# MIT-REALM/gcbfplus

Hardware: NVIDIA H100
Metric: env-steps/sec (agents x envs x steps/s) DoubleIntegrator n=512 (higher is better)
Workload: dtype f32

## Files before the change

gcbfplus_b200/csrc/gemm_tc_prod.cuh:

```cuda
#pragma once
#include "gemm_tc.cuh"
#include "gnn.cuh"

namespace gcbf {
namespace tc {

struct ProdArgs {
    gcbf_env_desc d;
    const float *W1, *b1, *agent, *goal, *hits;
    const int32_t *edge_recv, *edge_src;
    int clip_all;
};

struct ChainArgs {
    const float* bias_g;
    const float* avec;
    const float* cst;
    float* logits;
};

constexpr int L1_FLOATS = 9 * 256;

template <int ED>
__device__ __forceinline__ void load_l1_table(float* sW, const float* W1, const float* b1, int tid, int nthreads) {
    for (int i = tid; i < ED * 256; i += nthreads) sW[i] = W1[i];
    for (int i = tid; i < 3 * 256; i += nthreads) {
        const int t = i / 256, c = i % 256;
        sW[(ED + t) * 256 + c] = W1[(ED + t) * 256 + c] + W1[(ED + 3 + 2) * 256 + c] + b1[c];
    }
}

template <int ED>
__device__ __forceinline__ void produce_l1_kblock(uint8_t* st, int r, int half, int kb, bool row_ok, const float* sW,
                                                  const float (&f)[ED], int stype) {
#pragma unroll
    for (int cc = 0; cc < 4; ++cc) {
        const int c = half * 4 + cc;
        float v[4] = {0.f, 0.f, 0.f, 0.f};
        if (row_ok) {
            const int n = kb * BK + c * 4;
#pragma unroll
            for (int j = 0; j < 4; ++j) {
                float y = sW[(ED + stype) * 256 + n + j];
#pragma unroll
                for (int q = 0; q < ED; ++q) y = fmaf(f[q], sW[q * 256 + n + j], y);
                v[j] = fmaxf(y, 0.f);
            }
        }
        float4 h, l;
        split_tf32(make_float4(v[0], v[1], v[2], v[3]), h, l);
        const int off = swz(r, c);
        *reinterpret_cast<float4*>(st + off) = h;
        *reinterpret_cast<float4*>(st + PLANE + off) = l;
    }
}

__device__ __forceinline__ void drain_msg(const float (&d)[64], uint8_t* smem, int g, int wt, const float* bias,
                                          float* msg, int n_valid) {
    const int r0 = 64 * g + frag_row0(wt);
#pragma unroll
    for (int i = 0; i < 64; i += 2) {
        const int r = r0 + 8 * ((i >> 1) & 1);
        const int c = frag_col(wt, i);
        const float2 o = make_float2(d[i] + bias[c], d[i + 1] + bias[c + 1]);
        if (r < n_valid) *reinterpret_cast<float2*>(msg + (size_t)r * 128 + c) = o;
        const float2 h = make_float2(rn_tf32(o.x), rn_tf32(o.y));
        const float2 l = make_float2(rn_tf32(o.x - h.x), rn_tf32(o.y - h.y));
        const int off = (c >> 5) * 32768 + swz(r, (c & 31) >> 2) + (c & 3) * 4;
        *reinterpret_cast<float2*>(smem + off) = h;
        *reinterpret_cast<float2*>(smem + off + 16384) = l;
    }
}

__device__ __forceinline__ void chain_kblock(float (&d)[64], uint8_t* smem, int g, int kb2, int slot) {
    const uint32_t a_hi = smem_u32(smem + kb2 * 32768) + g * WG_ROWS_BYTES;
    const uint32_t b_hi = smem_u32(smem + 2 * STG + slot * 32768);
    mma_kblock(d, a_hi, a_hi + 16384, b_hi, b_hi + 16384, kb2 == 0);
}

template <int KIND>
__device__ __forceinline__ void edge_row_setup(const ProdArgs& pa, int m, bool row_ok, float (&f)[EnvTraits<KIND>::ED],
                                               int& stype) {
    using T = EnvTraits<KIND>;
    constexpr int ED = T::ED, SD = T::SD;
    const int A_tot = pa.d.n_graphs * pa.d.n_agents;
#pragma unroll
    for (int c = 0; c < ED; ++c) f[c] = 0.f;
    stype = 0;
    if (row_ok) {
        const int a = min(max(pa.edge_recv[m], 0), A_tot - 1);
        const int code = min(pa.edge_src[m], A_tot - 1);
        float er[ED], es[ED], coef, nrm;
        edge_state_dev<KIND>(pa.agent + (size_t)a * SD, er);
        sender_state_dev<KIND>(code, a, pa.d.n_hits, pa.agent, pa.goal, pa.hits, es);
        edge_feat_dev<KIND>(er, es, pa.clip_all || code == -1, pa.d.comm_radius, f, &coef, &nrm);
        stype = (code >= 0) ? 2 : ((code == -1) ? 1 : 0);
    }
}

template <int ED>
__device__ __forceinline__ void edge_tile_mainloop(float (&d)[64], uint8_t* smem, uint64_t* full, uint64_t* empty,
                                                   uint32_t& it, int g, int r, int half, bool row_ok, const float* sW,
                                                   const float (&f)[ED], int stype) {
#pragma unroll
    for (int i = 0; i < 64; ++i) d[i] = 0.f;
    for (int kb = 0; kb < 8; ++kb, ++it) {
        const int s = it % STAGES;
        uint8_t* st = smem + s * STG;
        produce_l1_kblock<ED>(st, r, half, kb, row_ok, sW, f, stype);
        fence_async_smem();
        bar_wg(g);
        mbar_wait(&full[s], (it / STAGES) & 1);
        wg_fence();
        const uint32_t a_hi = smem_u32(st) + g * WG_ROWS_BYTES;
        mma_kblock(d, a_hi, a_hi + PLANE, smem_u32(st) + 2 * PLANE, smem_u32(st) + 3 * PLANE, kb == 0);
        wg_commit();
        wg_wait<1>();
        if (kb > 0) mbar_arrive(&empty[(it - 1) % STAGES]);
    }
    wg_wait<0>();
    mbar_arrive(&empty[(it - 1) % STAGES]);
}

template <int KIND>
__global__ void __launch_bounds__(THREADS_NN, 1)
edge_chain_kernel(const __grid_constant__ CUtensorMap tmBh, const __grid_constant__ CUtensorMap tmBl,
                  const __grid_constant__ CUtensorMap tmB2h, const __grid_constant__ CUtensorMap tmB2l,
                  const __grid_constant__ ProdArgs pa, const float* __restrict__ bias, float* __restrict__ C,
                  const int32_t* __restrict__ m_ptr, const int m_cap, const ChainArgs ch) {
    constexpr int ED = EnvTraits<KIND>::ED;
    extern __shared__ uint8_t smem_raw[];
    uint8_t* smem = smem_align1024(smem_raw);
    uint64_t* bars = reinterpret_cast<uint64_t*>(smem + STAGES * STG);
    uint64_t* full = bars;
    uint64_t* empty = bars + 3;
    uint64_t* b2_full = bars + 6;
    uint64_t* b2_empty = bars + 8;
    uint64_t* main_done = bars + 10;
    uint64_t* t2f = bars + 11;
    float* sW = reinterpret_cast<float*>(smem + STAGES * STG + 256);

    const int warp = threadIdx.x >> 5, lane = threadIdx.x & 31;
    if (threadIdx.x == 0) {
        for (int s = 0; s < 3; ++s) {
            mbar_init(&full[s], 1);
            mbar_init(&empty[s], CONSUMERS);
        }
        for (int i = 0; i < 2; ++i) {
            mbar_init(&b2_full[i], 1);
            mbar_init(&b2_empty[i], CONSUMERS);
        }
        mbar_init(main_done, CONSUMERS);
        mbar_init(t2f, CONSUMERS);
        asm volatile("fence.mbarrier_init.release.cluster;" ::: "memory");
    }
    load_l1_table<ED>(sW, pa.W1, pa.b1, threadIdx.x, blockDim.x);
    __syncthreads();
    const int M = min(*m_ptr, m_cap);
    const int n_tiles = (M + BM - 1) / BM;

    if (warp == 8) {
        if (lane == 0) {
            uint32_t it = 0, tc_ = 0;
            for (int tile = blockIdx.x; tile < n_tiles; tile += gridDim.x, ++tc_) {
                if (tc_ > 0) mbar_wait(t2f, (tc_ - 1) & 1);
                for (int kb = 0; kb < 8; ++kb, ++it) {
                    const int s = it % STAGES;
                    mbar_wait(&empty[s], ((it / STAGES) & 1) ^ 1);
                    uint8_t* st = smem + s * STG;
                    mbar_expect_tx(&full[s], 2 * PLANE);
                    tma_load_2d(st + 2 * PLANE, &tmBh, &full[s], kb * BK, 0);
                    tma_load_2d(st + 3 * PLANE, &tmBl, &full[s], kb * BK, 0);
                }
                mbar_wait(main_done, tc_ & 1);
                for (int kb2 = 0; kb2 < 4; ++kb2) {
                    const uint32_t j2 = tc_ * 4 + kb2, slot = j2 & 1, use = j2 >> 1;
                    mbar_wait(&b2_empty[slot], (use & 1) ^ 1);
                    uint8_t* sl = smem + 2 * STG + slot * 32768;
                    mbar_expect_tx(&b2_full[slot], 32768);
                    tma_load_2d(sl, &tmB2h, &b2_full[slot], kb2 * BK, 0);
                    tma_load_2d(sl + 16384, &tmB2l, &b2_full[slot], kb2 * BK, 0);
                }
            }
        }
        return;
    }
    const int g = warp >> 2, wt = threadIdx.x & 127;
    const int r = 64 * g + (wt & 63), half = wt >> 6;
    uint32_t it = 0, tc_ = 0;
    for (int tile = blockIdx.x; tile < n_tiles; tile += gridDim.x, ++tc_) {
        const int m0 = tile * BM;
        float f[ED];
        int stype;
        edge_row_setup<KIND>(pa, m0 + r, m0 + r < M, f, stype);
        float d[64];
        edge_tile_mainloop<ED>(d, smem, full, empty, it, g, r, half, m0 + r < M, sW, f, stype);
        mbar_arrive(main_done);
        bar_consumers();
        drain_msg(d, smem, g, wt, bias, C + (size_t)m0 * 128, M - m0);
        fence_async_smem();
        bar_wg(g);
        float d2[64];
#pragma unroll
        for (int i = 0; i < 64; ++i) d2[i] = 0.f;
        for (int kb2 = 0; kb2 < 4; ++kb2) {
            const uint32_t j2 = tc_ * 4 + kb2, slot = j2 & 1, use = j2 >> 1;
            mbar_wait(&b2_full[slot], use & 1);
            wg_fence();
            chain_kblock(d2, smem, g, kb2, slot);
            wg_commit();
            wg_wait<0>();
            mbar_arrive(&b2_empty[slot]);
        }
        float q[2][1];
        frag_relu_dot<1>(d2, ch.bias_g, ch.avec, 1, 1, wt, q);
        if ((lane & 3) == 0) {
            const int rr = m0 + 64 * g + frag_row0(wt);
            if (rr < M) ch.logits[rr] = q[0][0] + ch.cst[0];
            if (rr + 8 < M) ch.logits[rr + 8] = q[1][0] + ch.cst[0];
        }
        mbar_arrive(t2f);
        bar_consumers();
    }
}

constexpr int PROD_SMEM = STAGES * STG + 256 + L1_FLOATS * 4 + 1024;

inline int32_t launch_edge_msg(const gcbf_env_desc* d, const float* W1, const float* b1, const float* agent,
                               const float* goal, const float* hits, const int32_t* edge_recv,
                               const int32_t* edge_src, const int32_t* counters, int clip_all, const float* Bt_hi,
                               const float* Bt_lo, const float* bias, float* msg, cudaStream_t st,
                               const float* gate_Bt_hi, const float* gate_Bt_lo, const ChainArgs& chain) {
    if (!counters) {
        set_error("launch_edge_msg: the chained gate GEMM needs the device edge counter");
        return -1;
    }
    ProdArgs pa;
    memset(&pa, 0, sizeof(pa));
    pa.d = *d;
    pa.W1 = W1; pa.b1 = b1; pa.agent = agent; pa.goal = goal; pa.hits = hits;
    pa.edge_recv = edge_recv; pa.edge_src = edge_src; pa.clip_all = clip_all;
    const int K = 256, N = 128;
    CUtensorMap tmB, tmBl, tmG, tmGl;
    if (int32_t r = make_map(&tmB, Bt_hi, N, K, N)) return r;
    if (int32_t r = make_map(&tmBl, Bt_lo, N, K, N)) return r;
    if (int32_t r = make_map(&tmG, gate_Bt_hi, 128, 128, 128)) return r;
    if (int32_t r = make_map(&tmGl, gate_Bt_lo, 128, 128, 128)) return r;
    const int grid = min((d->edge_cap + BM - 1) / BM, sm_count());
    GCBF_DISPATCH_ENV(d->env_kind, {
        auto kern = edge_chain_kernel<KIND>;
        static bool attr_done = false;
        if (!attr_done) {
            cudaFuncSetAttribute(kern, cudaFuncAttributeMaxDynamicSharedMemorySize, PROD_SMEM);
            attr_done = true;
        }
        kern<<<grid, THREADS_NN, PROD_SMEM, st>>>(tmB, tmBl, tmG, tmGl, pa, bias, msg, counters, d->edge_cap, chain);
        count_launch();
        return check_launch("edge_chain_kernel");
// ... 7 lines not shown
```

gcbfplus_b200/csrc/rollout_persist.cu:

```cuda
#include <stdlib.h>

#include "gemm_tc_prod.cuh"
#include "geometry_dev.cuh"
#include "gnn.cuh"

namespace gcbf {
namespace rp {
using namespace tc;

constexpr int PT = 512;
constexpr int PW = PT / 32;
constexpr int STG = 65536;
constexpr int MAX_N = 512;
constexpr int MAX_OBS = 32;

enum { B_FULL = 0, B_EMPTY = 3, B_B2F = 6, B_B2E = 8, B_MAIN = 10, B_T2F = 11, B_COUNT = 12 };

constexpr int PNU = 2;
enum {
    K_B23 = 0,
    K_BIAS_G = 128,
    K_AVEC = 256,
    K_BU1 = 384,
    K_BU1ROW = 640,
// ... 5 lines not shown
};

struct PArgs {
    gcbf_env_desc d;
    int T, cap_env, C;
    const float *W1, *b1, *b23, *bias_g, *avec, *cst, *b_u1, *b_u1row, *buh, *ho, *bho;
    const float *goal, *obstacles, *ray_table;
    float *agent, *hits, *actions, *rewards, *costs;
    int32_t* counters;
    int32_t *row_start, *row_deg, *edge_recv, *edge_src;
    float *msg, *logit, *ag, *v1, *z;
    unsigned long long* prof;
    int soft;
    unsigned* gbar;
};

__device__ __forceinline__ unsigned long long gtime() {
    unsigned long long t;
    asm volatile("mov.u64 %0, %%globaltimer;" : "=l"(t));
    return t;
}
__device__ __forceinline__ void cluster_sync_all() {
    __syncwarp();
    asm volatile("barrier.cluster.arrive.release.aligned;\n\tbarrier.cluster.wait.acquire.aligned;" ::: "memory");
}
__device__ __forceinline__ void soft_group_sync(unsigned* ctr, unsigned target) {
    __syncthreads();
    if (threadIdx.x == 0) {
        __threadfence();
        atomicAdd(ctr, 1u);
        unsigned v;
        const unsigned long long t0 = global_ns();
        do {
            asm volatile("ld.acquire.gpu.global.u32 %0, [%1];" : "=r"(v) : "l"(ctr) : "memory");
            if (v < target && global_ns() - t0 > MBAR_TIMEOUT_NS) __trap();
        } while (v < target);
        __threadfence();
    }
    __syncthreads();
}
__device__ __forceinline__ void fence_async_global() { asm volatile("fence.proxy.async.global;" ::: "memory"); }
template <int KIND>
__global__ void __launch_bounds__(PT, 1)
rollout_persist_kernel(const __grid_constant__ PArgs P, const __grid_constant__ CUtensorMap tmW23h,
                       const __grid_constant__ CUtensorMap tmW23l, const __grid_constant__ CUtensorMap tmA1h,
                       const __grid_constant__ CUtensorMap tmA1l, const __grid_constant__ CUtensorMap tmU1h,
                       const __grid_constant__ CUtensorMap tmU1l, const __grid_constant__ CUtensorMap tmUHh,
                       const __grid_constant__ CUtensorMap tmUHl, const __grid_constant__ CUtensorMap tmAG,
                       const __grid_constant__ CUtensorMap tmV1) {
    using TR = EnvTraits<KIND>;
    constexpr int SD = TR::SD, ED = TR::ED, NU = TR::NU, PD = TR::PD;
    static_assert(PD == 2 && NU == PNU, "persistent rollout kernel: 2-D environments");
    constexpr int OBW = 16, OBS2 = OBS2D;
    constexpr int A_BYTES = 16384, B_BYTES = 16384;
    extern __shared__ uint8_t smem_raw[];
    uint8_t* smem = smem_align1024(smem_raw);
    uint64_t* bars = reinterpret_cast<uint64_t*>(smem + 3 * STG);
    int* s_tot = reinterpret_cast<int*>(smem + 3 * STG + 256 + 16);
    float* sW = reinterpret_cast<float*>(smem + 3 * STG + 512);
    float* sst = sW + 7 * 256;
    float* sobs = sst + MAX_N * 4;
    float* stab = sobs + MAX_OBS * OBS2;
    unsigned* sbits = reinterpret_cast<unsigned*>(stab + 64);
    int* s_off = reinterpret_cast<int*>(sbits + 64 * 16);
    unsigned* s_hb = reinterpret_cast<unsigned*>(s_off + 72);
    float* s_red = reinterpret_cast<float*>(s_hb + 64);
    float* sk = s_red + 3 * PW;

    const gcbf_env_desc& d = P.d;
    const int tid = threadIdx.x, warp = tid >> 5, lane = tid & 31;
    const int C = P.C;
    const bool soft = P.soft != 0;
    const int rank = (int)(blockIdx.x % C);
    const int env = blockIdx.x / C;
    const int L = soft ? 2 : C;
    const int lrank = rank % L, grp = rank / L;
    unsigned n_sync = 0;
#define SYNC_LOCAL() cluster_sync_all()
#define SYNC_ENV()                                                     \
    do {                                                               \
        if (soft) {                                                    \
            ++n_sync;                                                  \
            soft_group_sync(P.gbar + env, n_sync * (unsigned)C);       \
        } else {                                                       \
            cluster_sync_all();                                        \
        }                                                              \
    } while (0)
    const int N = d.n_agents, E = d.n_graphs, O = d.n_obs, R = d.n_hits, cap = P.cap_env;
    const int A_tot = E * N;
    const int APC = (N + C - 1) / C;
    const int a_lo = min(rank * APC, N), a_hi = min(a_lo + APC, N);
    const int n_words = (N + 31) / 32;
    const size_t env_e0 = (size_t)env * cap;
    const int env_a0 = env * N;
    const int seg_cap = cap / (C / L);
    const int seg_off = grp * seg_cap;
    const int ga_lo = min(grp * L * APC, N), ga_hi = min(ga_lo + L * APC, N);

    if (tid == 0) {
        for (int s = 0; s < 3; ++s) {
            mbar_init(&bars[B_FULL + s], 1);
            mbar_init(&bars[B_EMPTY + s], CONSUMERS);
        }
        for (int i = 0; i < 2; ++i) {
            mbar_init(&bars[B_B2F + i], 1);
            mbar_init(&bars[B_B2E + i], CONSUMERS);
        }
        mbar_init(&bars[B_MAIN], CONSUMERS);
        mbar_init(&bars[B_T2F], CONSUMERS);
        asm volatile("fence.mbarrier_init.release.cluster;" ::: "memory");
    }
    for (int i = tid; i < ED * 256; i += PT) sW[i] = P.W1[i];
    for (int i = tid; i < 3 * 256; i += PT) {
        const int t = i / 256, c = i % 256;
        sW[(ED + t) * 256 + c] = P.W1[(ED + t) * 256 + c] + P.W1[(ED + 3 + 2) * 256 + c] + P.b1[c];
    }
    auto stage = [&](int off, const float* src, int n) {
        for (int i = tid; i < n; i += PT) sk[off + i] = src[i];
    };
    stage(K_B23, P.b23, 128);
    stage(K_BIAS_G, P.bias_g, 128);
    stage(K_AVEC, P.avec, 128);
    stage(K_BU1, P.b_u1, 256);
    stage(K_BU1ROW, P.b_u1row, 256);
    stage(K_BUH, P.buh, 256);
    stage(K_HO, P.ho, 256 * NU);
    stage(K_BHO, P.bho, NU);
    stage(K_CST, P.cst, 1);
    if (O > 0) {
        const float* ob = P.obstacles + (d.obs_per_graph ? (size_t)env * O * OBW : 0);
        for (int i = tid; i < O * OBW; i += PT) sobs[(i / OBW) * OBS2 + (i % OBW)] = ob[i];
    }
    for (int i = tid; i < d.n_rays * PD; i += PT) stab[i] = P.ray_table[i];
    __syncthreads();
    derive_far_fields(sobs, O, d.comm_radius, tid, PT);
    uint32_t it = 0;
    uint32_t ne = 0;
    int M_cur = 0;
    SYNC_LOCAL();
    if (P.prof != nullptr && rank == 0 && tid == 0) P.prof[(size_t)(P.T + 1) * 8 + 2 * env] = gtime();

    for (int t = -1; t < P.T; ++t) {
        const int b = t & 1;
        const float* agent_t = P.agent + (size_t)max(t, 0) * A_tot * SD;
        const float* hits_t = P.hits + (size_t)max(t, 0) * A_tot * R * PD;
        const int32_t* rs_t = P.row_start + (size_t)b * A_tot;
        const int32_t* rd_t = P.row_deg + (size_t)b * A_tot;
        const int32_t* er_t = P.edge_recv + (size_t)b * E * cap;
        const int32_t* es_t = P.edge_src + (size_t)b * E * cap;
        const bool stamp = P.prof != nullptr && blockIdx.x == 0 && tid == 0;
        unsigned long long* pr = P.prof + (size_t)(t + 1) * 8;
        if (stamp) pr[0] = gtime();
        if (t >= 0) {
            const int n_tiles = (M_cur + BM - 1) / BM;
            const int my_tiles = (n_tiles > lrank) ? (n_tiles - lrank + L - 1) / L : 0;
            const size_t seg_e0 = env_e0 + seg_off;
            if (warp == 0) {
                if (lane == 0) {
                    uint32_t it_l = it, ne_l = ne;
                    for (int tile = lrank; tile < n_tiles; tile += L, ++ne_l) {
                        if (ne_l > 0) mbar_wait(&bars[B_T2F], (ne_l - 1) & 1);
                        for (int kb = 0; kb < 8; ++kb, ++it_l) {
                            const int s = it_l % 3;
                            mbar_wait(&bars[B_EMPTY + s], ((it_l / 3) & 1) ^ 1);
                            uint8_t* st = smem + s * STG;
                            mbar_expect_tx(&bars[B_FULL + s], 2 * B_BYTES);
                            tma_load_2d(st + 2 * A_BYTES, &tmW23h, &bars[B_FULL + s], kb * BK, 0);
                            tma_load_2d(st + 2 * A_BYTES + B_BYTES, &tmW23l, &bars[B_FULL + s], kb * BK, 0);
                        }
                        mbar_wait(&bars[B_MAIN], ne_l & 1);
                        for (int kb2 = 0; kb2 < 4; ++kb2) {
                            const uint32_t j2 = ne_l * 4 + kb2, slot = j2 & 1, use = j2 >> 1;
                            mbar_wait(&bars[B_B2E + slot], (use & 1) ^ 1);
                            uint8_t* sl = smem + 2 * STG + slot * 32768;
                            mbar_expect_tx(&bars[B_B2F + slot], 32768);
                            tma_load_2d(sl, &tmA1h, &bars[B_B2F + slot], kb2 * BK, 0);
                            tma_load_2d(sl + 16384, &tmA1l, &bars[B_B2F + slot], kb2 * BK, 0);
                        }
                    }
                }
            } else if (warp >= 8) {
                const int g = (warp - 8) >> 2, wt = tid & 127;
                const int r = 64 * g + (wt & 63), half = wt >> 6;
                uint32_t it_l = it, ne_l = ne;
                for (int tile = lrank; tile < n_tiles; tile += L, ++ne_l) {
                    const int ml = tile * BM + r;
                    const bool row_ok = ml < M_cur;
                    float f[ED];
                    int stype = 0;
#pragma unroll
                    for (int c = 0; c < ED; ++c) f[c] = 0.f;
                    if (row_ok) {
                        const int a = min(max(er_t[seg_e0 + ml], env_a0), env_a0 + N - 1);
                        const int code = min(es_t[seg_e0 + ml], env_a0 + N - 1);
                        float er[ED], es[ED], coef, nrm;
                        edge_state_dev<KIND>(sst + (size_t)(a - env_a0) * SD, er);
                        if (code >= 0) edge_state_dev<KIND>(sst + (size_t)(max(code, env_a0) - env_a0) * SD, es);
                        else sender_state_dev<KIND>(code, a, R, agent_t, P.goal, hits_t, es);
                        edge_feat_dev<KIND>(er, es, code == -1, d.comm_radius, f, &coef, &nrm);
                        stype = (code >= 0) ? 2 : ((code == -1) ? 1 : 0);
                    }
                    float dacc[64];
                    edge_tile_mainloop<ED>(dacc, smem, &bars[B_FULL], &bars[B_EMPTY], it_l, g, r, half, row_ok, sW, f, stype);
                    mbar_arrive(&bars[B_MAIN]);
                    bar_consumers();
                    drain_msg(dacc, smem, g, wt, sk + K_B23, P.msg + (seg_e0 + (size_t)tile * BM) * 128, M_cur - tile * BM);
                    fence_async_smem();
                    bar_wg(g);
                    float d2[64];
#pragma unroll
                    for (int i = 0; i < 64; ++i) d2[i] = 0.f;
                    for (int kb2 = 0; kb2 < 4; ++kb2) {
                        const uint32_t j2 = ne_l * 4 + kb2, slot = j2 & 1, use = j2 >> 1;
                        mbar_wait(&bars[B_B2F + slot], use & 1);
                        wg_fence();
                        chain_kblock(d2, smem, g, kb2, slot);
                        wg_commit();
                        wg_wait<0>();
                        mbar_arrive(&bars[B_B2E + slot]);
                    }
                    float q[2][1];
                    frag_relu_dot<1>(d2, sk + K_BIAS_G, sk + K_AVEC, 1, 1, wt, q);
                    if ((lane & 3) == 0) {
                        const int rr = tile * BM + 64 * g + frag_row0(wt);
                        if (rr < M_cur) P.logit[seg_e0 + rr] = q[0][0] + sk[K_CST];
                        if (rr + 8 < M_cur) P.logit[seg_e0 + rr + 8] = q[1][0] + sk[K_CST];
                    }
                    mbar_arrive(&bars[B_T2F]);
                    bar_consumers();
                }
            }
            it += 8u * my_tiles;
            ne += my_tiles;
            SYNC_LOCAL();
            if (stamp) pr[1] = gtime();

            for (int il = a_lo + warp; il < a_hi; il += PW) {
                const int a = env_a0 + il;
                const int rs = rs_t[a];
                int rd = rd_t[a];
                if (rs < 0 || rs + rd > cap) rd = 0;
                *reinterpret_cast<float4*>(P.ag + (size_t)a * 128 + lane * 4) =
                    aggregate_logits(rs, rd, P.logit + env_e0, P.msg + env_e0 * 128, lane);
            }
            fence_async_global();
            SYNC_LOCAL();
            if (stamp) pr[2] = gtime();

            const int n_items = ((ga_hi - ga_lo + BM - 1) / BM) * 2;
            const int my_items = (n_items > lrank) ? (n_items - lrank + L - 1) / L : 0;
            float* z_t = P.z + (size_t)(t & 1) * 2 * A_tot * 4;
#pragma unroll 1
            for (int ph2 = 0; ph2 < 2; ++ph2) {
                const int nkb = ph2 == 0 ? 4 : 8;
                const CUtensorMap* tmA = ph2 == 0 ? &tmAG : &tmV1;
                const CUtensorMap* tmBh = ph2 == 0 ? &tmU1h : &tmUHh;
                const CUtensorMap* tmBl = ph2 == 0 ? &tmU1l : &tmUHl;
                if (warp == 0) {
                    if (lane == 0) {
                        uint32_t it_l = it;
                        fence_async_global();
                        for (int item = lrank; item < n_items; item += L) {
                            const int m0 = ga_lo + (item >> 1) * BM, nc0 = (item & 1) * 128;
                            for (int kb = 0; kb < nkb; ++kb, ++it_l) {
                                const int s = it_l % 3;
                                mbar_wait(&bars[B_EMPTY + s], ((it_l / 3) & 1) ^ 1);
                                uint8_t* st = smem + s * STG;
                                mbar_expect_tx(&bars[B_FULL + s], A_BYTES + 2 * B_BYTES);
                                tma_load_2d(st, tmA, &bars[B_FULL + s], kb * BK, env_a0 + m0);
                                tma_load_2d(st + 2 * A_BYTES, tmBh, &bars[B_FULL + s], kb * BK, nc0);
                                tma_load_2d(st + 2 * A_BYTES + B_BYTES, tmBl, &bars[B_FULL + s], kb * BK, nc0);
                            }
                        }
                    }
                } else if (warp >= 8) {
                    const int g = (warp - 8) >> 2, wt = tid & 127;
                    uint32_t it_l = it;
                    for (int item = lrank; item < n_items; item += L) {
                        float dacc[64];
                        tma_a_mainloop(dacc, smem, &bars[B_FULL], &bars[B_EMPTY], it_l, nkb, g, wt);
                        const int m0 = ga_lo + (item >> 1) * BM, nc0 = (item & 1) * 128;
                        const int r0 = m0 + 64 * g + frag_row0(wt);
                        if (ph2 == 0) {
#pragma unroll
                            for (int i = 0; i < 64; i += 2) {
                                const int ml = r0 + 8 * ((i >> 1) & 1);
                                if (ml >= ga_hi) continue;
                                const int n = nc0 + frag_col(wt, i);
                                float2 o = make_float2(dacc[i], dacc[i + 1]);
                                const float2 bb = *reinterpret_cast<const float2*>(sk + K_BU1 + n);
                                o.x += bb.x; o.y += bb.y;
                                const float2 b2 = *reinterpret_cast<const float2*>(sk + K_BU1ROW + n);
                                o.x += b2.x; o.y += b2.y;
                                o.x = fmaxf(o.x, 0.f); o.y = fmaxf(o.y, 0.f);
                                *reinterpret_cast<float2*>(P.v1 + (size_t)(env_a0 + ml) * 256 + n) = o;
                            }
                        } else {
                            float q[2][4];
                            frag_relu_dot<4>(dacc, sk + K_BUH + nc0, sk + K_HO + nc0 * NU, NU, NU, wt, q);
                            if ((lane & 3) == 0)
#pragma unroll
                                for (int h = 0; h < 2; ++h)
                                    if (r0 + 8 * h < ga_hi)
                                        *reinterpret_cast<float4*>(z_t + ((size_t)(item & 1) * A_tot + env_a0 + r0 + 8 * h) * 4) =
                                            make_float4(q[h][0], q[h][1], q[h][2], q[h][3]);
                        }
                    }
                }
                it += (uint32_t)nkb * my_items;
                if (ph2 == 0) fence_async_global();
                if (ph2 == 0) SYNC_LOCAL();
                else SYNC_ENV();
                if (stamp) pr[3 + ph2] = gtime();
            }
        }

        {
            const int tn = t + 1;
            float* agent_n = P.agent + (size_t)tn * A_tot * SD;
            float* hits_n = P.hits + (size_t)tn * A_tot * R * PD;
            const int bn_ = tn & 1;
            int32_t* rs_n = P.row_start + (size_t)bn_ * A_tot;
            int32_t* rd_n = P.row_deg + (size_t)bn_ * A_tot;
            int32_t* er_n = P.edge_recv + (size_t)bn_ * E * cap;
            int32_t* es_n = P.edge_src + (size_t)bn_ * E * cap;
            if (t < 0) {
                for (int i = tid; i < N; i += PT) {
                    const float* a = agent_n + (size_t)(env_a0 + i) * SD;
#pragma unroll
                    for (int c = 0; c < SD; ++c) sst[i * SD + c] = a[c];
                }
            } else {
                const bool rec = rank == 0;
                float acc[3] = {0.f, 0.f, 0.f};
                float* act_t = P.actions + (size_t)t * A_tot * NU;
                for (int i = tid; i < N; i += PT) {
                    const size_t a = (size_t)env_a0 + i;
                    float zz[4] = {0.f, 0.f, 0.f, 0.f};
                    const float* z_t = P.z + (size_t)(t & 1) * 2 * A_tot * 4;
                    for (int p = 0; p < 2; ++p) {
                        const float4 v = *reinterpret_cast<const float4*>(z_t + ((size_t)p * A_tot + a) * 4);
                        zz[0] += v.x; zz[1] += v.y; zz[2] += v.z; zz[3] += v.w;
                    }
                    float x[SD], gl[SD], ur[NU], act[NU], xn[SD];
#pragma unroll
                    for (int c = 0; c < SD; ++c) {
                        x[c] = sst[i * SD + c];
                        gl[c] = P.goal[a * SD + c];
                    }
                    policy_action<KIND>(d, x, gl, zz, sk + K_BHO, ur, act);
                    if (rec)
#pragma unroll
                        for (int c = 0; c < NU; ++c) act_t[a * NU + c] = act[c];
                    const float sq = step_agent<KIND>(d, x, gl, act, ur, true, xn);
#pragma unroll
                    for (int c = 0; c < SD; ++c) sst[i * SD + c] = xn[c];
                    if (rec) {
#pragma unroll
                        for (int c = 0; c < SD; ++c) agent_n[a * SD + c] = xn[c];
                        const float nr = sqrtf(sq);
                        const bool col = collides_prev<PD, SD>(x, rs_t[a], rd_t[a], es_t + env_e0, agent_t, d.two_r);
                        bool in_obs = false;
                        if (O > 0) {
                            const float* ob = P.obstacles + (d.obs_per_graph ? (size_t)env * O * OBW : 0);
                            in_obs = inside_any<PD>(ob, O, x, d.radius);
                        }
                        acc[0] += nr * nr;
                        acc[1] += col ? 1.f : 0.f;
                        acc[2] += in_obs ? 1.f : 0.f;
                    }
                }
                if (rec) reduce_reward_cost<PW>(acc, s_red, N, P.rewards + (size_t)t * E + env, P.costs + (size_t)t * E + env);
            }
            __syncthreads();
            if (stamp) pr[5] = gtime();

            const int n_slots = a_hi - a_lo;
            for (int slot0 = 0; slot0 < APC; slot0 += PW) {
                const int slot = slot0 + warp;
                const int i = a_lo + slot;
                const bool valid = slot < n_slots;
                const int ii = valid ? i : 0;
                float p[PD];
#pragma unroll
                for (int c = 0; c < PD; ++c) p[c] = sst[ii * SD + c];
                const size_t a_glob = (size_t)env_a0 + ii;
                float* my_hits = hits_n + a_glob * R * PD;
                if (valid) lidar2d_warp(p, stab, sobs, O, d.n_rays, R, lane, my_hits);
                __syncwarp();
                const unsigned hit_bits = active_hit_bits<PD>(d, p, my_hits, lane, valid);
                int cnt = 0;
                if (valid) cnt = neighbour_bits<PD, SD>(d, p, i, sst, lane, sbits + slot * n_words);
                if (lane == 0 && slot < APC) {
                    s_off[slot + 1] = valid ? (1 + cnt + __popc(hit_bits)) : 0;
                    s_hb[slot] = hit_bits;
                }
            }
            __syncthreads();
            if (warp == 0) {
                int v0 = (lane < APC) ? s_off[lane + 1] : 0;
                int v1 = (lane + 32 < APC) ? s_off[lane + 33] : 0;
                int inc0 = v0, inc1 = v1;
#pragma unroll
                for (int o = 1; o < 32; o <<= 1) {
                    const int n0_ = __shfl_up_sync(0xffffffffu, inc0, o);
                    const int n1_ = __shfl_up_sync(0xffffffffu, inc1, o);
                    if (lane >= o) { inc0 += n0_; inc1 += n1_; }
                }
                const int tot0 = __shfl_sync(0xffffffffu, inc0, 31);
                __syncwarp();
                if (lane == 0) s_off[0] = 0;
                if (lane < APC) s_off[lane + 1] = inc0;
                if (lane + 32 < APC) s_off[lane + 33] = tot0 + inc1;
                __syncwarp();
                const int total = s_off[APC];
                if (lane < L) {
                    uint32_t ra;
                    asm volatile("mapa.shared::cluster.u32 %0, %1, %2;" : "=r"(ra) : "r"(smem_u32(&s_tot[lrank])), "r"(lane));
                    asm volatile("st.shared::cluster.u32 [%0], %1;" ::"r"(ra), "r"(total) : "memory");
                }
            }
            SYNC_LOCAL();
            if (stamp) pr[6] = gtime();
            int base = 0, env_total = 0;
            for (int r2 = 0; r2 < L; ++r2) {
                const int v = s_tot[r2];
                base += (r2 < lrank) ? v : 0;
                env_total += v;
            }
            for (int slot = warp; slot < n_slots; slot += PW) {
                const int i = a_lo + slot;
                const int a_id = env_a0 + i;
                const int deg = s_off[slot + 1] - s_off[slot];
                const bool over = base + s_off[slot] + deg > seg_cap;
                const int rbase = seg_off + base + s_off[slot];
                if (over) {
                    if (lane == 0) {
                        atomicOr(&P.counters[(size_t)tn * 4 + 1], 1);
                        rs_n[a_id] = 0;
                        rd_n[a_id] = 0;
                    }
                    continue;
                }
                if (lane == 0) {
                    rs_n[a_id] = rbase;
                    rd_n[a_id] = deg;
                }
                fill_row(er_n + env_e0, es_n + env_e0, rbase, a_id, env_a0, sbits + slot * n_words, n_words, s_hb[slot], lane);
            }
            if (lrank == 0 && tid == 0) atomicAdd(&P.counters[(size_t)tn * 4 + 0], min(env_total, seg_cap));
            M_cur = min(env_total, seg_cap);
            SYNC_LOCAL();
            if (stamp) pr[7] = gtime();
        }
    }
#undef SYNC_LOCAL
#undef SYNC_ENV
    if (P.prof != nullptr && rank == 0 && tid == 0) P.prof[(size_t)(P.T + 1) * 8 + 2 * env + 1] = gtime();
}

struct WsLayout {
    int64_t msg, logit, ag, v1, z, row_start, row_deg, edge_recv, edge_src, gbar, total;
};
static WsLayout make_ws_layout(int E, int N, int cap_env) {
    WsLayout W;
    int64_t o = 0;
    auto take = [&](int64_t n) { int64_t r = o; o += (n + 63) & ~(int64_t)63; return r; };
    const int64_t A = (int64_t)E * N, EC = (int64_t)E * cap_env;
    W.msg = take(EC * 128);
    W.logit = take(EC);
    W.ag = take(A * 128 + 128 * 128);
    W.v1 = take(A * 256 + 128 * 256);
    W.z = take(2 * 2 * A * 4);
    W.row_start = take(2 * A);
    W.row_deg = take(2 * A);
    W.edge_recv = take(2 * EC);
    W.edge_src = take(2 * EC);
    W.gbar = take(E);
    W.total = o;
    return W;
}
static int cluster_size(int N, int cap_env) {
    const int items = ((N + 127) / 128) * 2;
    const int tiles = (min(cap_env, 3 * N) + 127) / 128;
    int c = 1;
    while (c < 8 && c < max(items, tiles)) c <<= 1;
    return c;
}

}
}

using namespace gcbf;

extern "C" __attribute__((visibility("default"))) int64_t gcbf_rollout_persistent_workspace_floats(const gcbf_env_desc* desc) {
    if (!desc || desc->edge_cap <= 0 || desc->n_graphs <= 0 || desc->n_agents <= 0) return -1;
    return rp::make_ws_layout(desc->n_graphs, desc->n_agents, desc->edge_cap / desc->n_graphs).total + 64;
}

extern "C" __attribute__((visibility("default"))) int32_t gcbf_rollout_persistent_max_clusters(int32_t cluster_size);

extern "C" __attribute__((visibility("default"))) int32_t gcbf_rollout_persistent_supported(const gcbf_env_desc* desc) {
    if (!desc) return 0;
    const bool ok = desc->env_kind >= 0 && desc->env_kind <= 2 && desc->n_agents >= 1 && desc->n_agents <= rp::MAX_N &&
                    desc->n_obs <= rp::MAX_OBS && desc->n_rays <= 32 && desc->n_hits == desc->n_rays && desc->n_graphs >= 1 &&
                    desc->edge_cap / desc->n_graphs >= desc->n_agents && (desc->obs_per_graph == 1 || desc->n_obs == 0);
    if (!ok) return 0;
    const int C = rp::cluster_size(desc->n_agents, desc->edge_cap / desc->n_graphs);
    static int cached[9] = {0, 0, 0, 0, 0, 0, 0, 0, 0};
    if (cached[C] == 0) {
        const int n = gcbf_rollout_persistent_max_clusters(C);
        cached[C] = n > 0 ? n : -1;
    }
    if (cached[C] > 0 && desc->n_graphs <= cached[C]) return 2;
    if (cached[2] == 0) {
        const int n = gcbf_rollout_persistent_max_clusters(2);
        cached[2] = n > 0 ? n : -1;
    }
    if (C >= 2 && desc->n_graphs * C <= sm_count() && desc->n_graphs * (C / 2) <= cached[2]) return 2;
    return 1;
}

static int persist_smem_bytes() {
    return 3 * rp::STG + 512 + 7 * 256 * 4 + rp::MAX_N * 4 * 4 + rp::MAX_OBS * 24 * 4 + 64 * 4 + 64 * 16 * 4 + 72 * 4 + 64 * 4 +
           3 * rp::PW * 4 + rp::K_FLOATS * 4 + 1024;
}

extern "C" __attribute__((visibility("default"))) int32_t gcbf_rollout_persistent_max_clusters(int32_t cluster_size) {
    auto kern = rp::rollout_persist_kernel<GCBF_ENV_DOUBLE_INTEGRATOR>;
    const int smem = persist_smem_bytes();
    if (cudaFuncSetAttribute(kern, cudaFuncAttributeMaxDynamicSharedMemorySize, smem) != cudaSuccess) return -1;
    if (cluster_size > 8 &&
        cudaFuncSetAttribute(kern, cudaFuncAttributeNonPortableClusterSizeAllowed, 1) != cudaSuccess) return -1;
    cudaLaunchConfig_t cfg;
    memset(&cfg, 0, sizeof(cfg));
    cfg.gridDim = dim3((unsigned)(cluster_size * 64), 1, 1);
    cfg.blockDim = dim3(rp::PT, 1, 1);
    cfg.dynamicSmemBytes = smem;
    cudaLaunchAttribute attr[1];
    attr[0].id = cudaLaunchAttributeClusterDimension;
    attr[0].val.clusterDim.x = (unsigned)cluster_size;
    attr[0].val.clusterDim.y = 1;
    attr[0].val.clusterDim.z = 1;
// ... 127 lines not shown
```

gcbfplus_b200/csrc/geometry_dev.cuh:

```cuda
#pragma once
#include <math.h>

#include "common.cuh"

namespace gcbf {

static constexpr int GB_WARPS = 32;
#define NO_HIT 1e6f

__device__ __forceinline__ bool rect_inside(const float* ob, float px, float py, float r) {
    float rel_x = px - ob[0];
    float rel_y = py - ob[1];
    float rel_xx = fabsf(rel_x * ob[4] + rel_y * ob[5]) - ob[2];
    float rel_yy = fabsf(rel_x * ob[5] - rel_y * ob[4]) - ob[3];
    bool is_in_down = (rel_xx < r) && (rel_yy < 0.f);
    bool is_in_up = (rel_xx < 0.f) && (rel_yy < r);
    bool is_out_corner = (rel_xx > 0.f) && (rel_yy > 0.f);
    bool is_in_circle = sqrtf(rel_xx * rel_xx + rel_yy * rel_yy) < r;
    return (is_in_down || is_in_up) || (is_out_corner && is_in_circle);
}

__device__ __forceinline__ float nanmin(float a, float b) {
    return (isnan(a) || isnan(b)) ? NAN : fminf(a, b);
}

__device__ __forceinline__ float rect_raytrace(const float* ob, float x1, float y1, float x2, float y2) {
    float best = 0.f;
#pragma unroll
    for (int k = 0; k < 4; ++k) {
        const int kp = (k + 3) & 3;
        float x3 = ob[6 + 2 * k], y3 = ob[7 + 2 * k];
        float x4 = ob[6 + 2 * kp], y4 = ob[7 + 2 * kp];
        float det = (x1 - x2) * (y4 - y3) - (y1 - y2) * (x4 - x3);
        float sgn = (det > 0.f) ? 1.f : ((det < 0.f) ? -1.f : det);
        det = sgn * fminf(fmaxf(fabsf(det), 1e-7f), 1e7f);
        float alpha = ((y4 - y3) * (x1 - x3) - (x4 - x3) * (y1 - y3)) / det;
        float beta = (-(y1 - y2) * (x1 - x3) + (x1 - x2) * (y1 - y3)) / det;
        float v = ((alpha <= 1.f && alpha >= 0.f) && (beta <= 1.f && beta >= 0.f)) ? 1.f : 0.f;
        alpha = v * alpha + (1.f - v) * NO_HIT;
        best = (k == 0) ? alpha : nanmin(best, alpha);
    }
    return best;
}

__device__ __forceinline__ bool sphere_inside(const float* ob, float px, float py, float pz, float r) {
    float dx = px - ob[0], dy = py - ob[1], dz = pz - ob[2];
    return sqrtf(dx * dx + dy * dy + dz * dz) <= ob[3] + r;
}
__device__ __forceinline__ float sphere_raytrace(const float* ob, float x1, float y1, float z1, float x2,
                                                 float y2, float z2) {
    float dx = x2 - x1, dy = y2 - y1, dz = z2 - z1;
    float rmax = sqrtf(dx * dx + dy * dy + dz * dz);
    float A = rmax * rmax;
    float ex = x1 - ob[0], ey = y1 - ob[1], ez = z1 - ob[2];
    float B = 2.f * (dx * ex + dy * ey + dz * ez);
    float C = ex * ex + ey * ey + ez * ez - ob[3] * ob[3];
    float delta = B * B - 4.f * A * C;
    if (delta < 0.f && A > 1e-20f && fabsf(B) < 1e18f) return NO_HIT;
    float valid1 = (delta >= 0.f) ? 1.f : 0.f;
    float sq = sqrtf(delta * valid1);
    float alpha1 = (-B - sq) / (2.f * A) * valid1 + (1.f - valid1);
    float alpha2 = (-B + sq) / (2.f * A) * valid1 + (1.f - valid1);
    float a1 = ((alpha1 >= 0.f) ? 1.f : 0.f) * alpha1 + ((alpha1 < 0.f) ? 1.f : 0.f) * 1.f;
    float a2 = ((alpha2 >= 0.f) ? 1.f : 0.f) * alpha2 + ((alpha2 < 0.f) ? 1.f : 0.f) * 1.f;
    float alphas = fminf(a1, a2);
    alphas = fminf(fmaxf(alphas, 0.f), 1.f);
    return valid1 * alphas + (1.f - valid1) * NO_HIT;
}

template <int PD>
__device__ __forceinline__ bool inside_any(const float* sobs, int O, const float* p, float r) {
    bool in = false;
    if (PD == 2) {
        for (int o = 0; o < O; ++o) in = in || rect_inside(sobs + 16 * o, p[0], p[1], r);
    } else {
        for (int o = 0; o < O; ++o) in = in || sphere_inside(sobs + 4 * o, p[0], p[1], p[2], r);
    }
    return in;
}

struct SortKey {
    int flag;
    float alpha;
    int idx;
};
__device__ __forceinline__ bool key_less(const SortKey& a, const SortKey& b) {
    if (a.flag != b.flag) return a.flag < b.flag;
    if (a.flag == 0 && a.alpha != b.alpha) return a.alpha < b.alpha;
    return a.idx < b.idx;
}
__device__ __forceinline__ SortKey warp_sort32(SortKey k, int lane) {
#pragma unroll
    for (int size = 2; size <= 32; size <<= 1) {
#pragma unroll
        for (int j = size >> 1; j > 0; j >>= 1) {
            SortKey o;
            o.flag = __shfl_xor_sync(0xffffffffu, k.flag, j);
            o.alpha = __shfl_xor_sync(0xffffffffu, k.alpha, j);
            o.idx = __shfl_xor_sync(0xffffffffu, k.idx, j);
            const bool up = ((lane & size) == 0);
            const bool lower = ((lane & j) == 0);
            const bool keep_min = (up == lower);
            const bool o_less = key_less(o, k);
            if (keep_min ? o_less : !o_less) k = o;
        }
    }
    return k;
}

template <int KIND>
__device__ __forceinline__ void u_ref_dev(const gcbf_env_desc& d, const float* x, const float* gl, float* u) {
    using T = EnvTraits<KIND>;
    constexpr int SD = T::SD, NU = T::NU;
    if (KIND == GCBF_ENV_DUBINS_CAR) {
        const float PI_F = 3.14159265358979323846f;
        const float TWO_PI = 6.283185307179586f;
        const float pdx = x[0] - gl[0], pdy = x[1] - gl[1];
        const float dist = sqrtf(pdx * pdx + pdy * pdy);
        float theta_t = atan2f(-pdy, -pdx);
        theta_t = theta_t - floorf(theta_t / TWO_PI) * TWO_PI;
        float theta = x[2] - floorf(x[2] / TWO_PI) * TWO_PI;
        const float theta_diff = theta_t - theta;
        const float dot = (-pdx) * cosf(theta) + (-pdy) * sinf(theta);
        const float tb = acosf(fminf(fmaxf(dot / (dist + 0.0001f), -1.f), 1.f));
        float omega = 0.f;
        const bool c1 = (theta_diff < PI_F) && (theta_diff >= 0.f);
        if (c1 && theta <= PI_F) omega = 1.0f * tb;
        if (!c1 && theta <= PI_F) omega = -1.0f * tb;
        const bool c2 = (theta_diff > -PI_F) && (theta_diff <= 0.f);
        if (c2 && theta > PI_F) omega = -1.0f * tb;
        if (!c2 && theta > PI_F) omega = 1.0f * tb;
        omega = fminf(fmaxf(omega, -5.f), 5.f);
        const float nrm = sqrtf(1e-6f + (pdx * pdx + pdy * pdy));
        const float coef = (nrm > d.comm_radius) ? d.comm_radius / fmaxf(nrm, d.comm_radius) : 1.f;
        const float qx = coef * pdx, qy = coef * pdy;
        u[0] = omega;
        u[1] = -2.5f * x[3] + 2.3f * sqrtf(qx * qx + qy * qy);
        return;
    }
    float err[SD];
    float acc = 0.f;
#pragma unroll
    for (int c = 0; c < SD; ++c) {
        err[c] = gl[c] - x[c];
        acc = (c == 0) ? err[c] * err[c] : acc + err[c] * err[c];
    }
    const float nrm = sqrtf(acc);
#pragma unroll
    for (int c = 0; c < SD; ++c) {
        const float emax = fabsf(err[c] / nrm * d.comm_radius);
        float e = err[c];
        e = (isnan(e) || isnan(emax)) ? NAN : fminf(fmaxf(e, -emax), emax);
        err[c] = e;
    }
#pragma unroll
    for (int a = 0; a < NU; ++a) {
        float s = 0.f;
#pragma unroll
        for (int c = 0; c < SD; ++c) s = (c == 0) ? err[c] * d.K[a * SD + c] : s + err[c] * d.K[a * SD + c];
        u[a] = isnan(s) ? NAN : fminf(fmaxf(s, -d.u_lim), d.u_lim);
    }
}

template <int KIND>
__device__ __forceinline__ void euler_dev(const gcbf_env_desc& d, const float* x, const float* gl, const float* u,
                                          float* xn, const bool stop_mask = true) {
    using T = EnvTraits<KIND>;
    constexpr int SD = T::SD, NU = T::NU;
    float xd[SD];
    if (KIND == GCBF_ENV_SINGLE_INTEGRATOR) {
        xd[0] = u[0];
        xd[1] = u[1];
    } else if (KIND == GCBF_ENV_DOUBLE_INTEGRATOR) {
        xd[0] = x[2];
        xd[1] = x[3];
        xd[2] = u[0] / d.mass;
        xd[3] = u[1] / d.mass;
    } else if (KIND == GCBF_ENV_DUBINS_CAR) {
        const float ddx = x[0] - gl[0], ddy = x[1] - gl[1];
        const float stop = (stop_mask && sqrtf(ddx * ddx + ddy * ddy) < d.half_r) ? 1.f : 0.f;
        const float keep = 1.f - stop;
        xd[0] = (cosf(x[2]) * x[3]) * keep;
        xd[1] = (sinf(x[2]) * x[3]) * keep;
        xd[2] = (u[0] * 20.f) * keep;
        xd[3] = u[1] * keep;
    } else {
#pragma unroll
        for (int r = 0; r < SD; ++r) {
            float s = 0.f;
#pragma unroll
            for (int c = 0; c < SD; ++c) s += x[c] * d.A[r * SD + c];
            float t = 0.f;
#pragma unroll
            for (int c = 0; c < NU; ++c) t += u[c] * d.B[r * NU + c];
            xd[r] = s + t;
        }
    }
#pragma unroll
    for (int c = 0; c < SD; ++c) {
        float v = xd[c] * d.dt + x[c];
        const bool limited = (KIND == GCBF_ENV_DOUBLE_INTEGRATOR && c >= 2) || (KIND == GCBF_ENV_DUBINS_CAR && c == 3) ||
                             (KIND == GCBF_ENV_LINEAR_DRONE && c >= 3);
        if (limited) v = isnan(v) ? v : fminf(fmaxf(v, -d.v_lim), d.v_lim);
        xn[c] = v;
    }
}

template <int KIND>
__device__ __forceinline__ float step_agent(const gcbf_env_desc& d, const float* x, const float* gl, const float* act,
                                            const float* ur, const bool stop_mask, float* xn) {
    constexpr int NU = EnvTraits<KIND>::NU;
    float u[NU], sq = 0.f;
#pragma unroll
    for (int c = 0; c < NU; ++c) {
        u[c] = isnan(act[c]) ? act[c] : fminf(fmaxf(act[c], -d.u_lim), d.u_lim);
        const float df = u[c] - ur[c];
        sq = (c == 0) ? df * df : sq + df * df;
    }
    euler_dev<KIND>(d, x, gl, u, xn, stop_mask);
    return sq;
}

template <int KIND>
__device__ __forceinline__ void policy_action(const gcbf_env_desc& d, const float* x, const float* gl, const float* z,
                                              const float* bHO, float* ur, float* act) {
    u_ref_dev<KIND>(d, x, gl, ur);
#pragma unroll
    for (int c = 0; c < EnvTraits<KIND>::NU; ++c) act[c] = 2.f * tanhf(z[c] + bHO[c]) + ur[c];
}

template <int PD, int SD>
__device__ __forceinline__ bool collides_prev(const float* x, int rs, int rd, const int32_t* edge_src,
                                              const float* agent_prev, float two_r) {
    bool col = false;
    for (int e = rs + 1; e < rs + rd; ++e) {
        const int s = edge_src[e];
        if (s < 0) break;
        float dd = 0.f;
#pragma unroll
        for (int c = 0; c < PD; ++c) {
            const float dlt = x[c] - agent_prev[(size_t)s * SD + c];
            dd = (c == 0) ? dlt * dlt : dd + dlt * dlt;
        }
        col = col || (two_r > sqrtf(dd));
    }
    return col;
}

template <int NW>
__device__ __forceinline__ void reduce_reward_cost(const float* acc, float* s_red, int N, float* reward, float* cost) {
    const int lane = threadIdx.x & 31, warp = threadIdx.x >> 5;
#pragma unroll
    for (int q = 0; q < 3; ++q) {
        const float v = warp_sum(acc[q]);
        if (lane == 0) s_red[q * NW + warp] = v;
    }
    __syncthreads();
    if (threadIdx.x == 0) {
        float t[3] = {0.f, 0.f, 0.f};
        for (int w = 0; w < NW; ++w) {
            t[0] += s_red[0 * NW + w];
            t[1] += s_red[1 * NW + w];
            t[2] += s_red[2 * NW + w];
        }
        *reward = -(t[0] / (float)N);
        *cost = t[1] / (float)N + t[2] / (float)N;
    }
}

constexpr int OBS2D = 24;
__device__ __forceinline__ void derive_far_fields(float* sobs, int O, float comm_radius, int tid, int nthreads) {
    for (int o = tid; o < O; o += nthreads) {
        float* ob = sobs + OBS2D * o;
        const float reach = comm_radius + sqrtf(ob[2] * ob[2] + ob[3] * ob[3]) + 2e-3f;
        ob[14] = reach * reach;
#pragma unroll
        for (int k = 0; k < 4; ++k) {
            const int kp = (k + 3) & 3;
            ob[15 + k] = ob[6 + 2 * kp] - ob[6 + 2 * k];
            ob[19 + k] = ob[7 + 2 * kp] - ob[7 + 2 * k];
        }
    }
}

__device__ __forceinline__ void lidar2d_warp(const float* p, const float* stab, const float* sobs, int O, int n_rays,
                                             int R, int lane, float* my_hits) {
    const bool ray_ok = lane < n_rays;
    const int rl = ray_ok ? lane : 0;
    const float x1 = p[0], y1 = p[1];
    const float x2 = x1 + stab[rl * 2 + 0], y2 = y1 + stab[rl * 2 + 1];
    const float rdx = x1 - x2, rdy = y1 - y2;
    float alpha;
    if (O == 0) {
        alpha = 1.f * NO_HIT;
    } else {
        alpha = NO_HIT;
        bool is_in = false;
        for (int o = 0; o < O; ++o) {
            const float* ob = sobs + OBS2D * o;
            const float cx = x1 - ob[0], cy = y1 - ob[1];
            const bool far = (cx * cx + cy * cy) > ob[14];
            bool degenerate = false;
            if (far) {
#pragma unroll
                for (int k = 0; k < 4; ++k) {
                    const float det = rdx * ob[19 + k] - rdy * ob[15 + k];
                    degenerate = degenerate || !(det != 0.f);
                }
            }
            if (!far) is_in = is_in || rect_inside(ob, x1, y1, 0.f);
            if (!far || __any_sync(0xffffffffu, degenerate))
                alpha = nanmin(alpha, rect_raytrace(ob, x1, y1, x2, y2));
        }
        alpha = alpha * (1.f - (is_in ? 1.f : 0.f));
    }
    const float hx = x1 + (x2 - x1) * alpha;
    const float hy = y1 + (y2 - y1) * alpha;
    SortKey k;
    k.flag = ray_ok ? (isnan(alpha) ? 1 : 0) : 2;
    k.alpha = alpha;
    k.idx = lane;
    const bool all_miss = __all_sync(0xffffffffu, !ray_ok || alpha == NO_HIT);
    if (!all_miss) k = warp_sort32(k, lane);
    const float shx = __shfl_sync(0xffffffffu, hx, k.idx);
    const float shy = __shfl_sync(0xffffffffu, hy, k.idx);
    if (lane < R) {
        my_hits[lane * 2 + 0] = shx;
        my_hits[lane * 2 + 1] = shy;
    }
}

template <int PD>
__device__ __forceinline__ unsigned active_hit_bits(const gcbf_env_desc& d, const float* p, const float* my_hits, int lane,
                                                    bool valid) {
    bool act = false;
    if (valid && lane < d.n_hits) {
        float acc = 0.f;
#pragma unroll
        for (int c = 0; c < PD; ++c) {
            const float dlt = p[c] - my_hits[lane * PD + c];
            acc = (c == 0) ? dlt * dlt : acc + dlt * dlt;
        }
        act = acc < d.lidar_sq_thr;
    }
    return __ballot_sync(0xffffffffu, act);
}

template <int PD, int STRIDE>
__device__ __forceinline__ int neighbour_bits(const gcbf_env_desc& d, const float* p, int i, const float* pos, int lane,
                                              unsigned* my_bits) {
    const int N = d.n_agents;
    int cnt = 0;
    const int n_full = N >> 5;
#pragma unroll 4
    for (int w = 0; w < n_full; ++w) {
        const int j = (w << 5) + lane;
        float acc;
        if (PD == 2) {
            const float2 q = *reinterpret_cast<const float2*>(pos + j * STRIDE);
            const float dx = p[0] - q.x, dy = p[1] - q.y;
            acc = dx * dx;
            acc = acc + dy * dy;
        } else {
            acc = 0.f;
#pragma unroll
            for (int c = 0; c < PD; ++c) {
                const float dlt = p[c] - pos[j * STRIDE + c];
                acc = (c == 0) ? dlt * dlt : acc + dlt * dlt;
            }
        }
        unsigned bits = __ballot_sync(0xffffffffu, acc < d.comm_sq_thr);
        if (w == (i >> 5)) bits &= ~(1u << (i & 31));
        if (lane == 0) my_bits[w] = bits;
        cnt += __popc(bits);
    }
    if (N & 31) {
        const int j = (n_full << 5) + lane;
        bool ok = false;
        if (j < N && j != i) {
            float acc = 0.f;
#pragma unroll
            for (int c = 0; c < PD; ++c) {
                const float dlt = p[c] - pos[j * STRIDE + c];
                acc = (c == 0) ? dlt * dlt : acc + dlt * dlt;
            }
            ok = acc < d.comm_sq_thr;
        }
        const unsigned bits = __ballot_sync(0xffffffffu, ok);
        if (lane == 0) my_bits[n_full] = bits;
        cnt += __popc(bits);
    }
    return cnt;
}

__device__ __forceinline__ void fill_row(int32_t* er, int32_t* es, int rbase, int a_id, int sender0,
                                         const unsigned* my_bits, int n_words, unsigned hit_bits, int lane) {
    if (lane == 0) {
        er[rbase] = a_id;
        es[rbase] = -1;
    }
    int pos = rbase + 1;
    const unsigned lt = (1u << lane) - 1u;
    for (int w = 0; w < n_words; ++w) {
        const unsigned bits = my_bits[w];
        if (bits == 0u) continue;
        if ((bits >> lane) & 1u) {
            const int e = pos + __popc(bits & lt);
            er[e] = a_id;
            es[e] = sender0 + (w << 5) + lane;
        }
        pos += __popc(bits);
    }
    if ((hit_bits >> lane) & 1u) {
        const int e = pos + __popc(hit_bits & lt);
        er[e] = a_id;
        es[e] = -2 - lane;
    }
}

}
```

Baseline: 105.3 million.

## Distribute 64-row half tiles across CTAs for finer edge-GEMM load balance

```diff
diff --git a/gcbfplus_b200/csrc/gemm_tc_prod.cuh b/gcbfplus_b200/csrc/gemm_tc_prod.cuh
--- a/gcbfplus_b200/csrc/gemm_tc_prod.cuh
+++ b/gcbfplus_b200/csrc/gemm_tc_prod.cuh
@@ -98,12 +98,19 @@
     }
 }
 
-template <int ED>
+template <int ED, bool MAY_IDLE = false>
 __device__ __forceinline__ void edge_tile_mainloop(float (&d)[64], uint8_t* smem, uint64_t* full, uint64_t* empty,
                                                    uint32_t& it, int g, int r, int half, bool row_ok, const float* sW,
-                                                   const float (&f)[ED], int stype) {
+                                                   const float (&f)[ED], int stype, bool active = true) {
 #pragma unroll
     for (int i = 0; i < 64; ++i) d[i] = 0.f;
+    if (MAY_IDLE && !active) {
+        for (int kb = 0; kb < 8; ++kb, ++it) {
+            mbar_wait(&full[it % STAGES], (it / STAGES) & 1);
+            mbar_arrive(&empty[it % STAGES]);
+        }
+        return;
+    }
     for (int kb = 0; kb < 8; ++kb, ++it) {
         const int s = it % STAGES;
         uint8_t* st = smem + s * STG;
diff --git a/gcbfplus_b200/csrc/rollout_persist.cu b/gcbfplus_b200/csrc/rollout_persist.cu
--- a/gcbfplus_b200/csrc/rollout_persist.cu
+++ b/gcbfplus_b200/csrc/rollout_persist.cu
@@ -181,13 +181,14 @@
         unsigned long long* pr = P.prof + (size_t)(t + 1) * 8;
         if (stamp) pr[0] = gtime();
         if (t >= 0) {
-            const int n_tiles = (M_cur + BM - 1) / BM;
-            const int my_tiles = (n_tiles > lrank) ? (n_tiles - lrank + L - 1) / L : 0;
+            const int n_half = (M_cur + 63) / 64;
+            const int my_half = (n_half > lrank) ? (n_half - lrank + L - 1) / L : 0;
+            const int my_tiles = (my_half + 1) / 2;
             const size_t seg_e0 = env_e0 + seg_off;
             if (warp == 0) {
                 if (lane == 0) {
                     uint32_t it_l = it, ne_l = ne;
-                    for (int tile = lrank; tile < n_tiles; tile += L, ++ne_l) {
+                    for (int k = 0; k < my_tiles; ++k, ++ne_l) {
                         if (ne_l > 0) mbar_wait(&bars[B_T2F], (ne_l - 1) & 1);
                         for (int kb = 0; kb < 8; ++kb, ++it_l) {
                             const int s = it_l % 3;
@@ -212,9 +213,12 @@
                 const int g = (warp - 8) >> 2, wt = tid & 127;
                 const int r = 64 * g + (wt & 63), half = wt >> 6;
                 uint32_t it_l = it, ne_l = ne;
-                for (int tile = lrank; tile < n_tiles; tile += L, ++ne_l) {
-                    const int ml = tile * BM + r;
-                    const bool row_ok = ml < M_cur;
+                for (int k = 0; k < my_tiles; ++k, ++ne_l) {
+                    const int j = 2 * k + g;
+                    const bool active = j < my_half;
+                    const int h0 = 64 * (lrank + j * L);
+                    const int ml = h0 + (wt & 63);
+                    const bool row_ok = active && ml < M_cur;
                     float f[ED];
                     int stype = 0;
 #pragma unroll
@@ -230,10 +234,12 @@
                         stype = (code >= 0) ? 2 : ((code == -1) ? 1 : 0);
                     }
                     float dacc[64];
-                    edge_tile_mainloop<ED>(dacc, smem, &bars[B_FULL], &bars[B_EMPTY], it_l, g, r, half, row_ok, sW, f, stype);
+                    edge_tile_mainloop<ED, true>(dacc, smem, &bars[B_FULL], &bars[B_EMPTY], it_l, g, r, half, row_ok, sW, f,
+                                                 stype, active);
                     mbar_arrive(&bars[B_MAIN]);
                     bar_consumers();
-                    drain_msg(dacc, smem, g, wt, sk + K_B23, P.msg + (seg_e0 + (size_t)tile * BM) * 128, M_cur - tile * BM);
+                    drain_msg(dacc, smem, g, wt, sk + K_B23, P.msg + (seg_e0 + (size_t)(h0 - 64 * g)) * 128,
+                              M_cur - (h0 - 64 * g));
                     fence_async_smem();
                     bar_wg(g);
                     float d2[64];
@@ -242,16 +248,18 @@
                     for (int kb2 = 0; kb2 < 4; ++kb2) {
                         const uint32_t j2 = ne_l * 4 + kb2, slot = j2 & 1, use = j2 >> 1;
                         mbar_wait(&bars[B_B2F + slot], use & 1);
-                        wg_fence();
-                        chain_kblock(d2, smem, g, kb2, slot);
-                        wg_commit();
-                        wg_wait<0>();
+                        if (active) {
+                            wg_fence();
+                            chain_kblock(d2, smem, g, kb2, slot);
+                            wg_commit();
+                            wg_wait<0>();
+                        }
                         mbar_arrive(&bars[B_B2E + slot]);
                     }
                     float q[2][1];
                     frag_relu_dot<1>(d2, sk + K_BIAS_G, sk + K_AVEC, 1, 1, wt, q);
                     if ((lane & 3) == 0) {
-                        const int rr = tile * BM + 64 * g + frag_row0(wt);
+                        const int rr = h0 + frag_row0(wt);
                         if (rr < M_cur) P.logit[seg_e0 + rr] = q[0][0] + sk[K_CST];
                         if (rr + 8 < M_cur) P.logit[seg_e0 + rr + 8] = q[1][0] + sk[K_CST];
                     }
```

After: 107.0 million, median of 6. +1.6%, better.

## Read policy-tail collision and obstacle checks from shared memory, keep lidar hits in registers

Applied to the files above, without the earlier changes.

```diff
diff --git a/gcbfplus_b200/csrc/geometry_dev.cuh b/gcbfplus_b200/csrc/geometry_dev.cuh
--- a/gcbfplus_b200/csrc/geometry_dev.cuh
+++ b/gcbfplus_b200/csrc/geometry_dev.cuh
@@ -68,11 +68,11 @@
     return valid1 * alphas + (1.f - valid1) * NO_HIT;
 }
 
-template <int PD>
+template <int PD, int OSTRIDE = 16>
 __device__ __forceinline__ bool inside_any(const float* sobs, int O, const float* p, float r) {
     bool in = false;
     if (PD == 2) {
-        for (int o = 0; o < O; ++o) in = in || rect_inside(sobs + 16 * o, p[0], p[1], r);
+        for (int o = 0; o < O; ++o) in = in || rect_inside(sobs + OSTRIDE * o, p[0], p[1], r);
     } else {
         for (int o = 0; o < O; ++o) in = in || sphere_inside(sobs + 4 * o, p[0], p[1], p[2], r);
     }
@@ -231,7 +231,7 @@
 
 template <int PD, int SD>
 __device__ __forceinline__ bool collides_prev(const float* x, int rs, int rd, const int32_t* edge_src,
-                                              const float* agent_prev, float two_r) {
+                                              const float* agent_prev, float two_r, int sender0 = 0) {
     bool col = false;
     for (int e = rs + 1; e < rs + rd; ++e) {
         const int s = edge_src[e];
@@ -239,7 +239,7 @@
         float dd = 0.f;
 #pragma unroll
         for (int c = 0; c < PD; ++c) {
-            const float dlt = x[c] - agent_prev[(size_t)s * SD + c];
+            const float dlt = x[c] - agent_prev[(size_t)(s - sender0) * SD + c];
             dd = (c == 0) ? dlt * dlt : dd + dlt * dlt;
         }
         col = col || (two_r > sqrtf(dd));
@@ -283,8 +283,8 @@
     }
 }
 
-__device__ __forceinline__ void lidar2d_warp(const float* p, const float* stab, const float* sobs, int O, int n_rays,
-                                             int R, int lane, float* my_hits) {
+__device__ __forceinline__ float2 lidar2d_warp(const float* p, const float* stab, const float* sobs, int O, int n_rays,
+                                               int R, int lane, float* my_hits) {
     const bool ray_ok = lane < n_rays;
     const int rl = ray_ok ? lane : 0;
     const float x1 = p[0], y1 = p[1];
@@ -328,6 +328,7 @@
         my_hits[lane * 2 + 0] = shx;
         my_hits[lane * 2 + 1] = shy;
     }
+    return make_float2(shx, shy);
 }
 
 template <int PD>
@@ -341,6 +342,17 @@
             const float dlt = p[c] - my_hits[lane * PD + c];
             acc = (c == 0) ? dlt * dlt : acc + dlt * dlt;
         }
+        act = acc < d.lidar_sq_thr;
+    }
+    return __ballot_sync(0xffffffffu, act);
+}
+__device__ __forceinline__ unsigned active_hit_bits_2d(const gcbf_env_desc& d, const float* p, float2 hit, int lane,
+                                                       bool valid) {
+    bool act = false;
+    if (valid && lane < d.n_hits) {
+        const float dx = p[0] - hit.x, dy = p[1] - hit.y;
+        float acc = dx * dx;
+        acc = acc + dy * dy;
         act = acc < d.lidar_sq_thr;
     }
     return __ballot_sync(0xffffffffu, act);
diff --git a/gcbfplus_b200/csrc/rollout_persist.cu b/gcbfplus_b200/csrc/rollout_persist.cu
--- a/gcbfplus_b200/csrc/rollout_persist.cu
+++ b/gcbfplus_b200/csrc/rollout_persist.cu
@@ -360,10 +360,13 @@
                     for (int c = 0; c < SD; ++c) sst[i * SD + c] = a[c];
                 }
             } else {
+                static_assert(MAX_N <= PT, "policy tail: one agent per thread");
                 const bool rec = rank == 0;
                 float acc[3] = {0.f, 0.f, 0.f};
                 float* act_t = P.actions + (size_t)t * A_tot * NU;
-                for (int i = tid; i < N; i += PT) {
+                float xn[SD];
+                const int i = tid;
+                if (i < N) {
                     const size_t a = (size_t)env_a0 + i;
                     float zz[4] = {0.f, 0.f, 0.f, 0.f};
                     const float* z_t = P.z + (size_t)(t & 1) * 2 * A_tot * 4;
@@ -371,7 +374,7 @@
                         const float4 v = *reinterpret_cast<const float4*>(z_t + ((size_t)p * A_tot + a) * 4);
                         zz[0] += v.x; zz[1] += v.y; zz[2] += v.z; zz[3] += v.w;
                     }
-                    float x[SD], gl[SD], ur[NU], act[NU], xn[SD];
+                    float x[SD], gl[SD], ur[NU], act[NU];
 #pragma unroll
                     for (int c = 0; c < SD; ++c) {
                         x[c] = sst[i * SD + c];
@@ -382,24 +385,22 @@
 #pragma unroll
                         for (int c = 0; c < NU; ++c) act_t[a * NU + c] = act[c];
                     const float sq = step_agent<KIND>(d, x, gl, act, ur, true, xn);
-#pragma unroll
-                    for (int c = 0; c < SD; ++c) sst[i * SD + c] = xn[c];
                     if (rec) {
 #pragma unroll
                         for (int c = 0; c < SD; ++c) agent_n[a * SD + c] = xn[c];
                         const float nr = sqrtf(sq);
-                        const bool col = collides_prev<PD, SD>(x, rs_t[a], rd_t[a], es_t + env_e0, agent_t, d.two_r);
-                        bool in_obs = false;
-                        if (O > 0) {
-                            const float* ob = P.obstacles + (d.obs_per_graph ? (size_t)env * O * OBW : 0);
-                            in_obs = inside_any<PD>(ob, O, x, d.radius);
-                        }
+                        const bool col = collides_prev<PD, SD>(x, rs_t[a], rd_t[a], es_t + env_e0, sst, d.two_r, env_a0);
+                        const bool in_obs = (O > 0) && inside_any<PD, OBS2>(sobs, O, x, d.radius);
                         acc[0] += nr * nr;
                         acc[1] += col ? 1.f : 0.f;
                         acc[2] += in_obs ? 1.f : 0.f;
                     }
                 }
                 if (rec) reduce_reward_cost<PW>(acc, s_red, N, P.rewards + (size_t)t * E + env, P.costs + (size_t)t * E + env);
+                else __syncthreads();
+                if (i < N)
+#pragma unroll
+                    for (int c = 0; c < SD; ++c) sst[i * SD + c] = xn[c];
             }
             __syncthreads();
             if (stamp) pr[5] = gtime();
@@ -415,9 +416,9 @@
                 for (int c = 0; c < PD; ++c) p[c] = sst[ii * SD + c];
                 const size_t a_glob = (size_t)env_a0 + ii;
                 float* my_hits = hits_n + a_glob * R * PD;
-                if (valid) lidar2d_warp(p, stab, sobs, O, d.n_rays, R, lane, my_hits);
-                __syncwarp();
-                const unsigned hit_bits = active_hit_bits<PD>(d, p, my_hits, lane, valid);
+                float2 hit = make_float2(0.f, 0.f);
+                if (valid) hit = lidar2d_warp(p, stab, sobs, O, d.n_rays, R, lane, my_hits);
+                const unsigned hit_bits = active_hit_bits_2d(d, p, hit, lane, valid);
                 int cnt = 0;
                 if (valid) cnt = neighbour_bits<PD, SD>(d, p, i, sst, lane, sbits + slot * n_words);
                 if (lane == 0 && slot < APC) {
```

New measurement: 110.0 million before, 111.1 million after (median of 6 runs). About the same (+1.0%).
